# arnauqb/GradABM-JUNE

Hardware: NVIDIA B200
Metric: agent_timesteps_per_sec_fwd_bwd (higher is better)
Workload: dtype f32

## Files before the change

gradabm-june_b200/csrc/gj_kernels.cu:

```cuda
#include <cuda_runtime.h>
#include <math.h>
#include <stdint.h>
#include <stdio.h>
#include <stdlib.h>
#include <string.h>

#include "gj_device.cuh"
#include "gj_tiled.cuh"
#include "gj_lean.cuh"
#include "gj_pipe.cuh"

namespace gj {

static thread_local char g_err[512] = "";

static int fail(const char* what, cudaError_t e) {
  snprintf(g_err, sizeof(g_err), "%s: %s", what, cudaGetErrorString(e));
  return -2;
}
static int bad(const char* what) {
  snprintf(g_err, sizeof(g_err), "invalid argument: %s", what);
  return -1;
}
#define GJ_CHECK_LAUNCH(name)                         \
  do {                                                \
    cudaError_t _e = cudaGetLastError();              \
    if (_e != cudaSuccess) return fail(name, _e);     \
  } while (0)

enum KernelId {
  K_TRANSMISSION = 0, K_GROUP_SMALL_F, K_GROUP_CHUNK_F, K_GROUP_FIX_F, K_AGENT_FWD,
  K_AGENT_BWD, K_GROUP_SMALL_B, K_GROUP_CHUNK_B, K_GROUP_FIX_B, K_DBETA, K_AGENT_BWD_GATHER, K_CELL, K_OTHER, K_SEED,
  K_EXCHANGE, K_SEED_GRAD, K_COUNT
};
static const char* kKernelNames[K_COUNT] = {
  "transmission", "group_small<fwd>", "group_chunk<fwd>", "group_fix<fwd>", "agent_forward",
  "agent_backward", "group_small<bwd>", "group_chunk<bwd>", "group_fix<bwd>", "dbeta",
  "backward_gather", "cell_groups+gather", "other", "seeding", "boundary_exchange", "seed_label_grad"};
constexpr int kMaxProfiled = 16384;
struct Profiler {
  bool on = false;
  int n = 0;
  int64_t launches[K_COUNT] = {0};
  cudaEvent_t ev[kMaxProfiled][2];
  int id[kMaxProfiled];
  bool created = false;
};
static Profiler g_prof;
struct ProfScope {
  int slot = -1;
  cudaStream_t st;
  ProfScope(int kid, cudaStream_t s) : st(s) {
    g_prof.launches[kid]++;
// ... 605 lines not shown
  return (int)(w->n_tiles < g ? w->n_tiles : g);
}

static int g_pipe_on = -1;
static int pipe_flags() {
  if (g_pipe_on < 0) {
    const char* e = getenv("GJ_PIPE");
    g_pipe_on = (e && e[0] >= '0' && e[0] <= '7') ? (e[0] - '0') : 1;
    const char* c = getenv("GJ_K1C");
    if (c && c[0] == '0') g_pipe_on |= 4;
  }
  return g_pipe_on;
}
static bool pipe_enabled() { return (pipe_flags() & 1) != 0; }
static bool lookahead_enabled() { return (pipe_flags() & 3) == 3; }
static bool aligned16(const void* p) { return (((uintptr_t)p) & 15u) == 0; }
static bool pipe_aligned_fwd(const gj_world_desc* w, const LeanPlan& lp, const gj_fwd_io* io) {
  return aligned16(io->s) && aligned16(io->inf) && aligned16(io->tinf) && aligned16(io->cur) && aligned16(io->nxt) &&
         aligned16(io->ttn) && aligned16(io->T) && aligned16(io->Tq) && aligned16(w->ent1) && aligned16(w->cls) &&
         aligned16(w->orig_id) &&
         aligned16(lp.r_slot) && aligned16(lp.r_pc);
}
static bool pipe_aligned_bwd(const gj_world_desc* w, const LeanPlan& lp, const gj_bwd_io* io) {
  const void* ptrs[] = {io->s, io->inf, io->tinf, io->cur, io->nxt, io->ttn, io->tape_y0, io->tape_v, io->g_s_o,
                        io->g_inf_o, io->g_tinf_o, io->g_cur_o, io->g_nxt_o, io->g_ttn_o, io->prof4, io->g_inf,
                        io->g_tinf, io->T_in, io->w, io->wq, w->ent1, w->cls, lp.r_slot, lp.r_pc};
  for (const void* q : ptrs)
    if (!aligned16(q)) return false;
  return true;
}
// ... 35 lines not shown
  if (w->n_chunks > 0) {
    ProfScope ps(kBwd ? K_GROUP_CHUNK_B : K_GROUP_CHUNK_F, st);
    k_group_chunk<kBwd><<<blocks_for(w->n_chunks * 32, kBlock), kBlock, 0, st>>>(*w, *p, ch, beta, lprob, in0, in1,
                                                                              out_a, out_b, sc.part_a, sc.part_b);
    GJ_CHECK_LAUNCH("k_group_chunk");
  }
  if (w->n_big > 0) {
    ProfScope ps(kBwd ? K_GROUP_FIX_B : K_GROUP_FIX_F, st);
    k_group_fix<kBwd><<<blocks_for(w->n_big, kBlock), kBlock, 0, st>>>(*w, *p, ch, beta, sc.part_a, sc.part_b, out_a,
                                                                     out_b);
    GJ_CHECK_LAUNCH("k_group_fix");
  }
  return 0;
}

static int launch_cell_groups(const gj_world_desc* w, const gj_step_params* p, const Plan& pl, const float* beta,
                              float* out_scaled, float* out_plain, const Scratch& sc, cudaStream_t st,
                              const Batch& bt = kNoBatch) {
  if (pl.n_t2 == 0) return 0;
  int64_t maxG = 1;
  for (int j = 0; j < pl.n_t2; ++j) {
    const int t = p->nets[pl.t2_net[j]].type;
    const int64_t G = w->type_group_off[t + 1] - w->type_group_off[t];
    if (G > maxG) maxG = G;
  }
  ProfScope ps(K_CELL, st);
  launch_pdl(k_cell_groups, dim3(blocks_for(maxG, kBlock), pl.n_t2, bt.nb), dim3(kBlock), 0, st, *w, *p, pl, beta,
             (const float*)sc.tile_part, out_scaled, out_plain, bt);
  GJ_CHECK_LAUNCH("k_cell_groups");
  return 0;
}

static int launch_cell_gather(const gj_world_desc* w, const gj_step_params* p, const Plan& pl, const float* in_scaled,
                              const Scratch& sc, cudaStream_t st, const Batch& bt = kNoBatch) {
  if (pl.n_t2 == 0) return 0;
  int64_t maxC = 1;
  for (int j = 0; j < pl.n_t2; ++j) {
    const int t = p->nets[pl.t2_net[j]].type;
    if (w->n_cells[t] > maxC) maxC = w->n_cells[t];
  }
  ProfScope ps(K_CELL, st);
  launch_pdl(k_cell_gather, dim3(blocks_for(maxC, kBlock), pl.n_t2, bt.nb), dim3(kBlock), 0, st, *w, *p, pl, in_scaled,
             sc.cell_buf, bt);
  GJ_CHECK_LAUNCH("k_cell_gather");
  return 0;
}

static bool lean_plan(const gj_world_desc* w, const gj_step_params* p, const Plan& pl, LeanPlan* lp) {
  memset(lp, 0, sizeof(*lp));
  if (p->mode != GJ_MODE_STEP || p->phases != GJ_PHASE_ALL || p->exact_order) return false;
  if (p->n_nets <= 0 || pl.n_t1 > 1) return false;
  if (pl.n_generic > 0 && !w->ent1) return false;
  int64_t total = 0;
  for (int k = 0; k < p->n_nets; ++k) {
    const int kind = p->nets[k].kind, t = p->nets[k].type;
    total += w->type_group_off[t + 1] - w->type_group_off[t];
    if (pl.tier[k] == GJ_TIER_RANGE) {
// ... 20 lines not shown
    } else if (kind == GJ_KIND_HOUSEHOLD) {
      if (p->n_quar > 0) return false;
    } else if (kind != GJ_KIND_PLAIN) {
      return false;
    }
  }
  lp->n_cell = pl.n_t2;
  lp->has_generic = pl.n_generic > 0;
  lp->gen_base = total;
  return true;
}

static int launch_lean_group_pass(const gj_world_desc* w, const gj_step_params* p, const Plan& pl, const float* beta,
                                  const float* in, float* out_scaled, float* out_plain, const Scratch& sc, bool bwd,
                                  cudaStream_t st, const Batch& bt);
static int launch_lean_forward_sums(const gj_world_desc* w, const gj_step_params* p, const Plan& pl, const float* beta,
                                    const float* in, float* out_scaled, float* out_plain, const Scratch& sc,
                                    cudaStream_t st, const Batch& bt) {
  if (w->n_giant_chunks > 0) {
    gj_world_desc wg = *w;
    wg.n_small = 0;
    wg.n_chunks = w->n_giant_chunks;
    wg.n_big = w->n_giant_big;
    if (int e = launch_lean_group_pass(&wg, p, pl, beta, in, out_scaled, out_plain, sc, false, st, bt)) return e;
  }
  {
    ProfScope ps(K_GROUP_SMALL_F, st);
    Scatter sct{sc.sct_acc, sc.sct_dirty};
    GenericRanges gr;
    memset(&gr, 0, sizeof(gr));
    for (int t = 0; t < w->n_types; ++t)
      if (w->type_tier[t] == GJ_TIER_GENERIC && w->type_group_off[t + 1] > w->type_group_off[t]) {
        gr.first[gr.n] = w->type_group_off[t];
        gr.start[gr.n + 1] = gr.start[gr.n] + (w->type_group_off[t + 1] - w->type_group_off[t]);
        ++gr.n;
      }
    if (gr.n == 0) return 0;
    launch_pdl(k_lean_scatter_finalize, dim3(blocks_for(gr.start[gr.n], kBlock) * bt.nb), dim3(kBlock), 0, st, *w, *p, pl,
               gr, beta, in, sct, out_scaled, out_plain, bt);
    GJ_CHECK_LAUNCH("k_lean_scatter_finalize");
  }
  return 0;
}

static int launch_lean_group_pass(const gj_world_desc* w, const gj_step_params* p, const Plan& pl, const float* beta,
                                  const float* in, float* out_scaled, float* out_plain, const Scratch& sc, bool bwd,
                                  cudaStream_t st, const Batch& bt) {
  if (w->n_small > 0 || w->n_chunks > 0) {
    ProfScope ps(bwd ? K_GROUP_CHUNK_B : K_GROUP_CHUNK_F, st);
    const int chunk_blocks = w->n_chunks > 0 ? blocks_for(w->n_chunks * 32, kBlock) : 0;
    const int small_blocks = w->n_small > 0 ? blocks_for(w->n_small, kBlock) : 0;
    launch_pdl(k_lean_group_sums, dim3((chunk_blocks + small_blocks) * bt.nb), dim3(kBlock), 0, st, *w, *p, pl, beta, in,
               out_scaled, out_plain, sc.part_a, chunk_blocks, bt);
    GJ_CHECK_LAUNCH("k_lean_group_sums");
  }
  if (w->n_big > 0) {
    ProfScope ps(bwd ? K_GROUP_FIX_B : K_GROUP_FIX_F, st);
    launch_pdl(k_lean_group_fix, dim3(blocks_for(w->n_big * 32, kBlock) * bt.nb), dim3(kBlock), 0, st, *w, *p, pl, beta,
               (const float*)sc.part_a, out_scaled, out_plain, bt);
    GJ_CHECK_LAUNCH("k_lean_group_fix");
  }
  return 0;
}

static int lean_forward(const gj_world_desc* w, const gj_step_params* p, const Plan& pl, const LeanPlan& lp,
                        const gj_fwd_io* io, const Scratch& sc, cudaStream_t st, const NextStep* next,
                        const Batch& bt = kNoBatch) {
  const bool quar = p->n_quar > 0;
  const bool batch = bt.nb > 1;
  if (p->stage != GJ_STAGE_REST) {
    if (!p->t_ready) {
      ProfScope ps(K_TRANSMISSION, st);
      static OccCache occ[4];
      const Scatter sct{sc.sct_acc, sc.sct_dirty};
#define GJ_K1(Q, B, I)                                                                                               \
  launch_pdl(k_lean_transmission<Q, B>, dim3(lean_grid(w, k_lean_transmission<Q, B>, &occ[I], bt)), dim3(kLeanThreads), \
             0, st, *w, *p, lp, *io, sc.tile_part, sct, bt)
#define GJ_K1C(Q, B, I)                                                                                              \
  launch_pdl(k_lean_transmission_c<Q, B>, dim3(lean_grid(w, k_lean_transmission_c<Q, B>, &occ_c[I], bt)),              \
             dim3(kLeanThreads), 0, st, *w, *p, lp, *io, sc.tile_part, sct, bt)
      static OccCache occ_c[4];
      const bool compact = (pipe_flags() & 4) == 0;
      if (compact) {
        if (batch) {
// ... 2 lines not shown
        } else {
          if (quar) GJ_K1C(true, false, 1);
          else GJ_K1C(false, false, 0);
        }
      } else if (batch) {
        if (quar) GJ_K1(true, true, 3);
        else GJ_K1(false, true, 2);
      } else {
        if (quar) GJ_K1(true, false, 1);
        else GJ_K1(false, false, 0);
      }
#undef GJ_K1
#undef GJ_K1C
      GJ_CHECK_LAUNCH("k_lean_transmission");
    }
    if (lp.has_generic)
      if (int e = launch_lean_forward_sums(w, p, pl, io->beta, quar ? io->Tq : io->T, io->S_scaled + lp.gen_base,
                                           io->S_unscaled + lp.gen_base, sc, st, bt))
        return e;
    if (int e = launch_cell_groups(w, p, pl, io->beta, io->S_scaled, io->S_unscaled, sc, st, bt)) return e;
  }
  if (p->stage == GJ_STAGE_SUMS) return 0;
  if (int e = launch_cell_gather(w, p, pl, io->S_scaled, sc, st, bt)) return e;
  if (batch && bt.noise && pipe_enabled() && pipe_aligned_fwd(w, lp, io)) {
    ProfScope pn(K_OTHER, st);
    launch_pdl(k_batch_noise, dim3(agent_grid(w->n_agents)), dim3(kBlock), 0, st, *w, *p, const_cast<float*>(bt.noise));
    GJ_CHECK_LAUNCH("k_batch_noise");
  }
  if (pipe_enabled() && pipe_aligned_fwd(w, lp, io)) {
    ProfScope ps(K_AGENT_FWD, st);
    static OccCache occ[20];
    const bool diag = io->q || io->n;
    const bool lab = io->label != nullptr;
    const size_t smem = next ? sizeof(PipeFwdSharedT<true, false>)
                             : (batch ? sizeof(PipeFwdSharedT<false, true>) : sizeof(PipeFwdSharedT<false, false>));
    NextStep nx;
    memset(&nx, 0, sizeof(nx));
    if (next) {
// ... 56 lines not shown
    }
#undef GJ_LEAN_FWD
    GJ_CHECK_LAUNCH("k_lean_forward");
  }
  return 0;
}

static int lean_backward(const gj_world_desc* w, const gj_step_params* p, const Plan& pl, LeanPlan lp,
                         const gj_bwd_io* io, const Scratch& sc, cudaStream_t st, const Batch& bt = kNoBatch) {
  const bool quar = p->n_quar > 0;
  const bool batch = bt.nb > 1;
  static OccCache occ_b[4], occ_g[2];
  const bool lab = io->label && io->g_red_label;
  int gather_grid = 1;
  const bool pipe = pipe_enabled() && pipe_aligned_bwd(w, lp, io);
  if (batch && !pipe) return bad("batched step: the pipelined kernels are off or an array is not 16-byte aligned");
  if (p->stage != GJ_STAGE_REST) {
    if (pipe) {
      ProfScope ps(K_AGENT_BWD, st);
      static OccCache occ[8];
      const size_t smem = sizeof(PipeBwdShared);
#define GJ_PIPE_BWD(Q, B, L, I)                                                                                       \
  launch_pdl(k_pipe_backward<Q, B, L>, dim3(pipe_grid(w, k_pipe_backward<Q, B, L>, kBwdThreads, smem, &occ[I], bt)),    \
             dim3(kBwdThreads), smem, st, *w, *p, lp, *io, sc.tile_part, bt)
      if (lab && batch) {
        if (quar) GJ_PIPE_BWD(true, true, true, 7);
        else GJ_PIPE_BWD(false, true, true, 6);
      } else if (lab) {
        if (quar) GJ_PIPE_BWD(true, false, true, 5);
        else GJ_PIPE_BWD(false, false, true, 4);
// ... 8 lines not shown
      GJ_CHECK_LAUNCH("k_pipe_backward");
    } else {
      ProfScope ps(K_AGENT_BWD, st);
#define GJ_LEAN_BWD(Q, L, I) \
  k_lean_backward<Q, L><<<lean_grid(w, k_lean_backward<Q, L>, &occ_b[I]), kLeanThreads, 0, st>>>(*w, *p, lp, *io, sc.tile_part)
      if (lab) {
        if (quar) GJ_LEAN_BWD(true, true, 3);
        else GJ_LEAN_BWD(false, true, 2);
      } else {
        if (quar) GJ_LEAN_BWD(true, false, 1);
        else GJ_LEAN_BWD(false, false, 0);
      }
#undef GJ_LEAN_BWD
      GJ_CHECK_LAUNCH("k_lean_backward");
    }
    if (lp.has_generic)
      if (int e = launch_lean_group_pass(w, p, pl, io->beta, quar ? io->wq : io->w, io->cR + lp.gen_base,
                                         io->R + lp.gen_base, sc, true, st, bt))
        return e;
    if (int e = launch_cell_groups(w, p, pl, io->beta, io->cR, io->R, sc, st, bt)) return e;
  }
  if (p->stage == GJ_STAGE_SUMS) return 0;
  if (int e = launch_cell_gather(w, p, pl, io->cR, sc, st, bt)) return e;
  if (pipe) {
    ProfScope ps(K_AGENT_BWD_GATHER, st);
    static OccCache occ[4];
    const size_t smem = sizeof(PipeGatShared);
#define GJ_PIPE_GAT(Q, B, I)                                                                                          \
  launch_pdl(k_pipe_backward_gather<Q, B>,                                                                            \
             dim3(gather_grid = pipe_grid(w, k_pipe_backward_gather<Q, B>, kPipeThreads, smem, &occ[I], bt)),          \
             dim3(kPipeThreads), smem, st, *w, *p, lp, *io, (const float*)sc.cell_buf, sc.dbeta_tile, bt)
    if (batch) {
      if (quar) GJ_PIPE_GAT(true, true, 3);
      else GJ_PIPE_GAT(false, true, 2);
    } else {
      if (quar) GJ_PIPE_GAT(true, false, 1);
      else GJ_PIPE_GAT(false, false, 0);
    }
// ... 307 lines not shown
  }
  return err ? 1 : 0;
}

int gj_peer_destroy(gj_peer* p) {
  if (!p) return 0;
  for (int r = 0; r < p->world; ++r)
    if (r != p->rank && p->mapped[r]) cudaIpcCloseMemHandle(p->mapped[r]);
  cudaFree(p->own);
  delete p;
  return 0;
}

int gj_pipeline_enable(int on) {
  const int prev = pipe_flags();
  if (on >= 0) g_pipe_on = on & 7;
  return prev;
}

int gj_profile_enable(int on) {
  if (on && !g_prof.created) {
    for (int i = 0; i < kMaxProfiled; ++i) {
      if (cudaEventCreate(&g_prof.ev[i][0]) != cudaSuccess || cudaEventCreate(&g_prof.ev[i][1]) != cudaSuccess)
        return fail("cudaEventCreate", cudaGetLastError());
    }
    g_prof.created = true;
  }
  g_prof.on = on != 0;
  g_prof.n = 0;
  for (int i = 0; i < K_COUNT; ++i) g_prof.launches[i] = 0;
  return 0;
// ... 440 lines not shown
```

gradabm-june_b200/csrc/gj_lean.cuh:

```cuda
#pragma once
#include "gj_tiled.cuh"

namespace gj {

constexpr int kLeanThreads = 256;
#ifndef GJ_LEAN_MINB_FWD
#define GJ_LEAN_MINB_FWD 3
#endif
#ifndef GJ_LEAN_MINB_BWD
#define GJ_LEAN_MINB_BWD 4
#endif
#ifndef GJ_LEAN_MINB_GATHER
#define GJ_LEAN_MINB_GATHER 3
#endif
constexpr uint32_t kEntNone = 0xFFFFFFFFu;
constexpr uint32_t kEntMulti = 0xFFFFFFFEu;
constexpr uint32_t kEntGiant = 0x80000000u;
constexpr uint32_t kEntId = 0x7FFFFFFFu;

struct Scatter {
  unsigned long long* acc;
  uint8_t* dirty;
};
constexpr float kScatterScale = (float)(1ull << GJ_SCATTER_FRAC);
// ... 478 lines not shown
    bx /= (uint32_t)bt.nb;
    beta += (int64_t)s * bt.sBeta;
    in += (int64_t)s * bt.sN;
    out_scaled += (int64_t)s * bt.sG;
    out_plain += (int64_t)s * bt.sG;
    part = scr_shift(part, bt, s);
  }
  lean_beta_sums(gs, w, p, pl, beta);
  if ((int)bx < chunk_blocks)
    lean_group_chunk_body(w, gs, ((int64_t)bx * blockDim.x + threadIdx.x) >> 5, in, out_scaled, out_plain, part);
  else
    lean_group_small_body(w, gs, (int64_t)(bx - chunk_blocks) * blockDim.x + threadIdx.x, in, out_scaled,
                          out_plain);
}

__global__ void __launch_bounds__(kBlock) k_lean_group_fix(gj_world_desc w, gj_step_params p, Plan pl,
                                                           const float* __restrict__ beta,
                                                           const float* __restrict__ part,
                                                           float* __restrict__ out_scaled,
                                                           float* __restrict__ out_plain, Batch bt) {
  __shared__ LeanGroupShared gs;
  pdl_launch();
  pdl_wait();
  uint32_t bx = blockIdx.x;
  if (bt.nb > 1) {
    const int s = (int)(bx % (uint32_t)bt.nb);
    bx /= (uint32_t)bt.nb;
    beta += (int64_t)s * bt.sBeta;
    out_scaled += (int64_t)s * bt.sG;
    out_plain += (int64_t)s * bt.sG;
    part = scr_shift(part, bt, s);
  }
  lean_beta_sums(gs, w, p, pl, beta);
  const int lane = threadIdx.x & 31;
  const int64_t i = ((int64_t)bx * blockDim.x + threadIdx.x) >> 5;
  if (i >= w.n_big) return;
  const uint32_t g = w.big_groups[i];
  const float b = lean_group_beta(gs, g);
  float S = 0.0f;
  for (uint32_t j = w.big_part_ptr[i] + lane; j < w.big_part_ptr[i + 1]; j += 32) S += part[j];
  S = warp_sum(S);
  if (lane != 0) return;
  out_plain[g] = S;
  out_scaled[g] = (b == b) ? (b * w.pc[g]) * S : 0.0f;
}

struct GenericRanges {
  int n;
  int64_t first[GJ_MAX_TYPES];
  int64_t start[GJ_MAX_TYPES + 1];
};
__global__ void __launch_bounds__(kBlock) k_lean_scatter_finalize(gj_world_desc w, gj_step_params p, Plan pl,
                                                                  GenericRanges gr, const float* __restrict__ beta,
                                                                  const float* __restrict__ in, Scatter sct,
                                                                  float* __restrict__ out_scaled,
                                                                  float* __restrict__ out_plain, Batch bt) {
  __shared__ LeanGroupShared gs;
  pdl_launch();
  pdl_wait();
  uint32_t bx = blockIdx.x;
  if (bt.nb > 1) {
    const int s = (int)(bx % (uint32_t)bt.nb);
    bx /= (uint32_t)bt.nb;
    beta += (int64_t)s * bt.sBeta;
    in += (int64_t)s * bt.sN;
    out_scaled += (int64_t)s * bt.sG;
    out_plain += (int64_t)s * bt.sG;
    sct.acc = scr_shift(sct.acc, bt, s);
    sct.dirty = scr_shift(sct.dirty, bt, s);
  }
  lean_beta_sums(gs, w, p, pl, beta);
  const int64_t i = (int64_t)bx * blockDim.x + threadIdx.x;
  if (i >= gr.start[gr.n]) return;
  int r = 0;
#pragma unroll
  for (int k = 1; k < GJ_MAX_TYPES; ++k) r += (k < gr.n && i >= gr.start[k]) ? 1 : 0;
  const int64_t g = gr.first[r] + (i - gr.start[r]);
  const uint32_t j0 = w.gm_ptr[g], j1 = w.gm_ptr[g + 1];
  if (j1 - j0 > (uint32_t)GJ_SCATTER_MAX_GROUP) return;
  const unsigned long long acc = sct.acc[g];
  const bool dirty = sct.dirty[g] != 0;
  if (acc != 0ull) sct.acc[g] = 0ull;
  const float b = lean_group_beta(gs, (uint32_t)g);
  float S = (float)((double)(long long)acc * (1.0 / (double)(1ull << GJ_SCATTER_FRAC)));
  if (dirty) {
    sct.dirty[g] = 0;
    S = 0.0f;
    for (uint32_t j = j0; j < j1; ++j) S += in[w.gm_agent[j]];
  }
  out_plain[g] = S;
  out_scaled[g] = (b == b) ? (b * w.pc[g]) * S : 0.0f;
}

struct FwdOut {
  float inf, tinf, cur;
};
struct FwdRes {
  float tape_v, tape_y0, q, lam, n;
  float s_o, inf_o, tinf_o, cur_o, nxt_o, ttn_o;
};
__device__ __forceinline__ float lean_noise_dE(uint32_t r0, uint32_t r1) {
  return lg2_fast(fmaxf(-lg2_fast(u01_open(r0)), kMinE2)) - lg2_fast(fmaxf(-lg2_fast(u01_open(r1)), kMinE2));
}
template <bool kQuar>
__device__ __forceinline__ FwdRes lean_forward_core(const gj_step_params& p, const LeanPlan& lp,
                                                    const float* __restrict__ stage_prob, uint64_t ga, float dE,
// ... 569 lines not shown
```

gradabm-june_b200/csrc/gj_tiled.cuh:

```cuda
#pragma once
#include "gj_device.cuh"

namespace gj {

constexpr uint32_t kNoSlot = 0xFFFFFFFFu;

struct Plan {
  int n_t2;
  int t2_net[GJ_MAX_CHANNELS];
  int net_t2[GJ_MAX_NETS];
  int n_t1;
  int t1_net[GJ_MAX_RANGE_NETS];
  int net_t1[GJ_MAX_NETS];
  int n_lei;
  int lei_net[GJ_MAX_CHANNELS];
  int net_lei[GJ_MAX_NETS];
  int n_generic;
  int tier[GJ_MAX_NETS];
  const uint32_t* slot[GJ_MAX_NETS];
  const float* rpc[GJ_MAX_NETS];
};

struct Batch {
  int nb;
// ... 141 lines not shown
    float Tq = T;
    if (quar) {
      Tq = quarantine_mask(p, io.cur[a]) * T;
      io.Tq[a] = Tq;
    }
    if (pl.n_t2 > 0 && T != 0.0f) {
      const int cls = w.cls[a];
#pragma unroll
      for (int j = 0; j < GJ_MAX_CHANNELS; ++j)
        if (j < pl.n_t2) acc[j] += member_value(tb, pl, pl.t2_net[j], p.nets[pl.t2_net[j]].kind, T, Tq, cls);
    }
  }
  if (pl.n_t2 > 0) block_sums<float, GJ_MAX_CHANNELS>(acc, pl.n_t2, tile_part + tile * GJ_MAX_CHANNELS);
}

__global__ void __launch_bounds__(kBlock) k_cell_groups(gj_world_desc w, gj_step_params p, Plan pl,
                                                        const float* __restrict__ beta,
                                                        const float* __restrict__ tile_part,
                                                        float* __restrict__ out_scaled, float* __restrict__ out_plain,
                                                        Batch bt) {
  pdl_launch();
  pdl_wait();
  if (bt.nb > 1) {
    const int s = blockIdx.z;
    beta += (int64_t)s * bt.sBeta;
    tile_part = scr_shift(tile_part, bt, s);
    out_scaled += (int64_t)s * bt.sG;
    out_plain += (int64_t)s * bt.sG;
  }
  const int j = blockIdx.y;
  const int k = pl.t2_net[j];
  const gj_net net = p.nets[k];
  const int t = net.type;
  const int64_t G = w.type_group_off[t + 1] - w.type_group_off[t];
  const int64_t g = (int64_t)blockIdx.x * blockDim.x + threadIdx.x;
  if (g >= G) return;
  float sum = 0.0f;
  for (uint32_t ci = w.grp_cell_ptr[t][g]; ci < w.grp_cell_ptr[t][g + 1]; ++ci) {
    const uint32_t c = w.grp_cell[t][ci];
    for (uint32_t tl = w.cell_tile_ptr[t][c]; tl < w.cell_tile_ptr[t][c + 1]; ++tl)
      sum += tile_part[(int64_t)tl * GJ_MAX_CHANNELS + j];
  }
  const float cg = beta[k] * w.pc[w.type_group_off[t] + g];
  out_plain[(int64_t)net.s_off + g] = sum;
  out_scaled[(int64_t)net.s_off + g] = cg * sum;
}

__global__ void __launch_bounds__(kBlock) k_cell_gather(gj_world_desc w, gj_step_params p, Plan pl,
                                                        const float* __restrict__ in_scaled,
                                                        float* __restrict__ cell_buf, Batch bt) {
  pdl_launch();
  pdl_wait();
  if (bt.nb > 1) {
    const int s = blockIdx.z;
    in_scaled += (int64_t)s * bt.sG;
    cell_buf = scr_shift(cell_buf, bt, s);
  }
  const int j = blockIdx.y;
  const gj_net net = p.nets[pl.t2_net[j]];
  const int t = net.type;
  const int64_t c = (int64_t)blockIdx.x * blockDim.x + threadIdx.x;
  if (c >= w.n_cells[t]) return;
  float sum = 0.0f;
  for (uint32_t gi = w.cell_grp_ptr[t][c]; gi < w.cell_grp_ptr[t][c + 1]; ++gi)
    sum += in_scaled[(int64_t)net.s_off + w.cell_grp[t][gi]];
  cell_buf[(w.cell_off[t] + c) * GJ_MAX_CHANNELS + j] = sum;
}

struct AgentState {
  float s, inf, tinf, cur, nxt, ttn;
};

template <bool kLabel = false, bool kSeed = false>
__device__ __forceinline__ void forward_tail(const gj_step_params& p, const gj_fwd_io& io, int64_t N, int64_t a,
                                             int64_t ga, int age, float q, AgentState st, float* red,
                                             uint32_t* lacc = nullptr) {
  const int dead = p.n_stages - 1;
  if (p.mode == GJ_MODE_SEED) q = 1.0f - io.seed_fraction[kSeed ? io.seed_label[a] : 0] * 1.0f;
  float n = 0.0f;
  StepNoise nz;
  nz.E0 = nz.E1 = 1.0f;
// ... 446 lines not shown
```

gradabm-june_b200/grad_june/_lib.py:

```python
import ctypes as C
import os
import subprocess
from pathlib import Path

PKG_DIR = Path(__file__).resolve().parent
CSRC_DIR = PKG_DIR.parent / "csrc"
INCLUDE_DIR = PKG_DIR.parent.parent / "include"
LIB_PATH = Path(os.environ.get("GJ_LIB_PATH") or PKG_DIR / "libgradjune_b200.so")

GJ_MAX_TYPES = 8
GJ_MAX_NETS = 16
GJ_MAX_STAGES = 16
GJ_MAX_QUAR = 4
GJ_MAX_AGE_BINS = 8
GJ_MAX_CHANNELS = 8
GJ_ABI_VERSION = 12

KIND_PLAIN, KIND_HOUSEHOLD, KIND_LEISURE, KIND_CARE_VISIT = 0, 1, 2, 3
PHASE_NETWORKS, PHASE_SAMPLE, PHASE_INFECT, PHASE_SYMPTOMS, PHASE_ALL = 1, 2, 4, 8, 15
MODE_STEP, MODE_SEED = 0, 1
STAGE_ALL, STAGE_SUMS, STAGE_REST = 0, 1, 2

_u32p = C.c_void_p
_f32p = C.c_void_p
# ... 217 lines not shown
        raise GradJuneLibraryError(f"{what} failed ({rc}): {lib().gj_last_error().decode()}")


EXPORTED_SYMBOLS = [
    "gj_abi_version", "gj_last_error", "gj_config", "gj_scratch_bytes", "gj_profile_prepare", "gj_profile_pack",
    "gj_transmission_forward", "gj_transmission_backward", "gj_step_forward", "gj_step_forward_next", "gj_step_backward",
    "gj_step_forward_batch", "gj_step_backward_batch",
    "gj_philox_fill", "gj_philox_fill_at", "gj_step_plan", "gj_philox4x32_10", "gj_philox2x32_10", "gj_profile_enable", "gj_profile_read",
    "gj_profile_kernel_name", "gj_pipeline_enable", "gj_boundary_pack", "gj_boundary_unpack",
    "gj_peer_create", "gj_peer_handle", "gj_peer_connect", "gj_peer_exchange", "gj_peer_status", "gj_peer_destroy",
    "gj_world_build", "gj_world_build_host", "gj_world_descriptor", "gj_world_permutation", "gj_world_last_error",
    "gj_world_destroy", "gj_memcpy",
]


def pipeline_enable(on=True, lookahead=False, uncompacted=False):
    prev = lib().gj_pipeline_enable(-1 if on is None else ((1 if on else 0) | (2 if (on and lookahead) else 0)
                                                           | (4 if uncompacted else 0)))
    return bool(prev & 1), bool(prev & 2), bool(prev & 4)


def profile_enable(on=True):
    check(lib().gj_profile_enable(1 if on else 0), "gj_profile_enable")


def profile_read():
    n = 24
    ms, timed, launches = (C.c_double * n)(), (C.c_int64 * n)(), (C.c_int64 * n)()
    k = lib().gj_profile_read(ms, timed, launches, n)
    if k < 0:
        check(k, "gj_profile_read")
    return {lib().gj_profile_kernel_name(i).decode(): (ms[i], timed[i], launches[i]) for i in range(k)}
```

Before: 21.17 billion.

## Fuse group sums, cell groups and cell gather into one cooperative persistent kernel

Replaces the separate launches for chunked/small group sums, scatter finalize, cell groups, group fix and cell gather with a single cooperative kernel. Work is dispatched over virtual blocks in two phases separated by a grid-wide barrier. Finalize blocks are processed in pairs to overlap their loads. This is meant to cut launch and inter-kernel gaps, at the cost of a software grid barrier and occupancy-limited persistent scheduling. It is enabled by default for non-batched full-stage steps.

```diff
diff --git a/gradabm-june_b200/csrc/gj_kernels.cu b/gradabm-june_b200/csrc/gj_kernels.cu
--- a/gradabm-june_b200/csrc/gj_kernels.cu
+++ b/gradabm-june_b200/csrc/gj_kernels.cu
@@ -31,12 +31,13 @@
 enum KernelId {
   K_TRANSMISSION = 0, K_GROUP_SMALL_F, K_GROUP_CHUNK_F, K_GROUP_FIX_F, K_AGENT_FWD,
   K_AGENT_BWD, K_GROUP_SMALL_B, K_GROUP_CHUNK_B, K_GROUP_FIX_B, K_DBETA, K_AGENT_BWD_GATHER, K_CELL, K_OTHER, K_SEED,
-  K_EXCHANGE, K_SEED_GRAD, K_COUNT
+  K_EXCHANGE, K_SEED_GRAD, K_SUMS_F, K_SUMS_B, K_COUNT
 };
 static const char* kKernelNames[K_COUNT] = {
   "transmission", "group_small<fwd>", "group_chunk<fwd>", "group_fix<fwd>", "agent_forward",
   "agent_backward", "group_small<bwd>", "group_chunk<bwd>", "group_fix<bwd>", "dbeta",
-  "backward_gather", "cell_groups+gather", "other", "seeding", "boundary_exchange", "seed_label_grad"};
+  "backward_gather", "cell_groups+gather", "other", "seeding", "boundary_exchange", "seed_label_grad",
+  "sums<fwd>", "sums<bwd>"};
 constexpr int kMaxProfiled = 16384;
 struct Profiler {
   bool on = false;
@@ -672,6 +673,7 @@
 }
 static bool pipe_enabled() { return (pipe_flags() & 1) != 0; }
 static bool lookahead_enabled() { return (pipe_flags() & 3) == 3; }
+static bool fused_sums_enabled() { return (pipe_flags() & 8) == 0; }
 static bool aligned16(const void* p) { return (((uintptr_t)p) & 15u) == 0; }
 static bool pipe_aligned_fwd(const gj_world_desc* w, const LeanPlan& lp, const gj_fwd_io* io) {
   return aligned16(io->s) && aligned16(io->inf) && aligned16(io->tinf) && aligned16(io->cur) && aligned16(io->nxt) &&
@@ -737,33 +739,40 @@
   return 0;
 }
 
-static int launch_cell_groups(const gj_world_desc* w, const gj_step_params* p, const Plan& pl, const float* beta,
-                              float* out_scaled, float* out_plain, const Scratch& sc, cudaStream_t st,
-                              const Batch& bt = kNoBatch) {
-  if (pl.n_t2 == 0) return 0;
+static int cell_group_blocks(const gj_world_desc* w, const gj_step_params* p, const Plan& pl) {
   int64_t maxG = 1;
   for (int j = 0; j < pl.n_t2; ++j) {
     const int t = p->nets[pl.t2_net[j]].type;
     const int64_t G = w->type_group_off[t + 1] - w->type_group_off[t];
     if (G > maxG) maxG = G;
   }
-  ProfScope ps(K_CELL, st);
-  launch_pdl(k_cell_groups, dim3(blocks_for(maxG, kBlock), pl.n_t2, bt.nb), dim3(kBlock), 0, st, *w, *p, pl, beta,
-             (const float*)sc.tile_part, out_scaled, out_plain, bt);
-  GJ_CHECK_LAUNCH("k_cell_groups");
-  return 0;
-}
-
-static int launch_cell_gather(const gj_world_desc* w, const gj_step_params* p, const Plan& pl, const float* in_scaled,
-                              const Scratch& sc, cudaStream_t st, const Batch& bt = kNoBatch) {
-  if (pl.n_t2 == 0) return 0;
+  return blocks_for(maxG, kBlock);
+}
+static int cell_gather_blocks(const gj_world_desc* w, const gj_step_params* p, const Plan& pl) {
   int64_t maxC = 1;
   for (int j = 0; j < pl.n_t2; ++j) {
     const int t = p->nets[pl.t2_net[j]].type;
     if (w->n_cells[t] > maxC) maxC = w->n_cells[t];
   }
+  return blocks_for(maxC, kBlock);
+}
+
+static int launch_cell_groups(const gj_world_desc* w, const gj_step_params* p, const Plan& pl, const float* beta,
+                              float* out_scaled, float* out_plain, const Scratch& sc, cudaStream_t st,
+                              const Batch& bt = kNoBatch) {
+  if (pl.n_t2 == 0) return 0;
   ProfScope ps(K_CELL, st);
-  launch_pdl(k_cell_gather, dim3(blocks_for(maxC, kBlock), pl.n_t2, bt.nb), dim3(kBlock), 0, st, *w, *p, pl, in_scaled,
+  launch_pdl(k_cell_groups, dim3(cell_group_blocks(w, p, pl), pl.n_t2, bt.nb), dim3(kBlock), 0, st, *w, *p, pl, beta,
+             (const float*)sc.tile_part, out_scaled, out_plain, bt);
+  GJ_CHECK_LAUNCH("k_cell_groups");
+  return 0;
+}
+
+static int launch_cell_gather(const gj_world_desc* w, const gj_step_params* p, const Plan& pl, const float* in_scaled,
+                              const Scratch& sc, cudaStream_t st, const Batch& bt = kNoBatch) {
+  if (pl.n_t2 == 0) return 0;
+  ProfScope ps(K_CELL, st);
+  launch_pdl(k_cell_gather, dim3(cell_gather_blocks(w, p, pl), pl.n_t2, bt.nb), dim3(kBlock), 0, st, *w, *p, pl, in_scaled,
              sc.cell_buf, bt);
   GJ_CHECK_LAUNCH("k_cell_gather");
   return 0;
@@ -814,6 +823,17 @@
 static int launch_lean_group_pass(const gj_world_desc* w, const gj_step_params* p, const Plan& pl, const float* beta,
                                   const float* in, float* out_scaled, float* out_plain, const Scratch& sc, bool bwd,
                                   cudaStream_t st, const Batch& bt);
+static GenericRanges generic_ranges(const gj_world_desc* w) {
+  GenericRanges gr;
+  memset(&gr, 0, sizeof(gr));
+  for (int t = 0; t < w->n_types; ++t)
+    if (w->type_tier[t] == GJ_TIER_GENERIC && w->type_group_off[t + 1] > w->type_group_off[t]) {
+      gr.first[gr.n] = w->type_group_off[t];
+      gr.start[gr.n + 1] = gr.start[gr.n] + (w->type_group_off[t + 1] - w->type_group_off[t]);
+      ++gr.n;
+    }
+  return gr;
+}
 static int launch_lean_forward_sums(const gj_world_desc* w, const gj_step_params* p, const Plan& pl, const float* beta,
                                     const float* in, float* out_scaled, float* out_plain, const Scratch& sc,
                                     cudaStream_t st, const Batch& bt) {
@@ -827,14 +847,7 @@
   {
     ProfScope ps(K_GROUP_SMALL_F, st);
     Scatter sct{sc.sct_acc, sc.sct_dirty};
-    GenericRanges gr;
-    memset(&gr, 0, sizeof(gr));
-    for (int t = 0; t < w->n_types; ++t)
-      if (w->type_tier[t] == GJ_TIER_GENERIC && w->type_group_off[t + 1] > w->type_group_off[t]) {
-        gr.first[gr.n] = w->type_group_off[t];
-        gr.start[gr.n + 1] = gr.start[gr.n] + (w->type_group_off[t + 1] - w->type_group_off[t]);
-        ++gr.n;
-      }
+    const GenericRanges gr = generic_ranges(w);
     if (gr.n == 0) return 0;
     launch_pdl(k_lean_scatter_finalize, dim3(blocks_for(gr.start[gr.n], kBlock) * bt.nb), dim3(kBlock), 0, st, *w, *p, pl,
                gr, beta, in, sct, out_scaled, out_plain, bt);
@@ -863,11 +876,80 @@
   return 0;
 }
 
+constexpr int kSumsBarrier = 62;
+static_assert(1 + GJ_MAX_NETS <= kSumsBarrier && (kSumsBarrier + 2) * sizeof(unsigned int) <= 256,
+              "grid barrier words overlap the reduction tickets");
+static_assert(sizeof(gj_world_desc) + sizeof(gj_step_params) + sizeof(Plan) + sizeof(SumsPlan) <= 32764,
+              "k_lean_sums parameters exceed the 32 KB kernel parameter limit");
+static int launch_lean_sums(const gj_world_desc* w, const gj_step_params* p, const Plan& pl, const LeanPlan& lp,
+                            const float* beta, const float* in, float* scaled, float* plain, const Scratch& sc,
+                            bool bwd, cudaStream_t st) {
+  SumsPlan sp;
+  memset(&sp, 0, sizeof(sp));
+  sp.beta = beta;
+  sp.in = in;
+  sp.gen_scaled = scaled + lp.gen_base;
+  sp.gen_plain = plain + lp.gen_base;
+  sp.part = sc.part_a;
+  if (lp.has_generic) {
+    sp.n_chunks = bwd ? w->n_chunks : w->n_giant_chunks;
+    sp.n_big = bwd ? w->n_big : w->n_giant_big;
+    sp.chunk_blocks = sp.n_chunks > 0 ? blocks_for(sp.n_chunks * 32, kBlock) : 0;
+    sp.small_blocks = (bwd && w->n_small > 0) ? blocks_for(w->n_small, kBlock) : 0;
+    sp.fix_blocks = sp.n_big > 0 ? blocks_for(sp.n_big * 32, kBlock) : 0;
+    if (!bwd) {
+      sp.gr = generic_ranges(w);
+      sp.sct = Scatter{sc.sct_acc, sc.sct_dirty};
+      sp.fin_blocks = sp.gr.n > 0 ? blocks_for(sp.gr.start[sp.gr.n], kBlock) : 0;
+    }
+  }
+  sp.tile_part = sc.tile_part;
+  sp.cell_scaled = scaled;
+  sp.cell_plain = plain;
+  sp.cell_buf = sc.cell_buf;
+  if (pl.n_t2 > 0) {
+    sp.cg_blocks = cell_group_blocks(w, p, pl);
+    sp.cc_blocks = cell_gather_blocks(w, p, pl);
+  }
+  sp.bar = sc.tickets + kSumsBarrier;
+  const int64_t n1 = (int64_t)sp.chunk_blocks + sp.small_blocks + sp.fin_blocks + (int64_t)pl.n_t2 * sp.cg_blocks;
+  const int64_t n2 = (int64_t)sp.fix_blocks + (int64_t)pl.n_t2 * sp.cc_blocks;
+  if (n1 + n2 == 0) return 0;
+  if (n1 >= ((int64_t)1 << 31) || n2 >= ((int64_t)1 << 31)) return bad("too many groups for k_lean_sums");
+  static OccCache occ;
+  int& per_sm = occ.v[current_device()];
+  if (per_sm == 0) {
+    cudaError_t e = cudaOccupancyMaxActiveBlocksPerMultiprocessor(&per_sm, k_lean_sums, kBlock, 0);
+    if (e != cudaSuccess || per_sm < 1) {
+      per_sm = 0;
+      return e != cudaSuccess ? fail("occupancy of k_lean_sums", e) : bad("k_lean_sums does not fit on an SM");
+    }
+  }
+  int64_t grid = (int64_t)sm_count() * per_sm;
+  const int64_t work = n1 > n2 ? n1 : n2;
+  if (grid > work) grid = work;
+  ProfScope ps(bwd ? K_SUMS_B : K_SUMS_F, st);
+  cudaLaunchConfig_t cfg;
+  memset(&cfg, 0, sizeof(cfg));
+  cfg.gridDim = dim3((unsigned)grid);
+  cfg.blockDim = dim3(kBlock);
+  cfg.stream = st;
+  cudaLaunchAttribute attr[1];
+  attr[0].id = cudaLaunchAttributeCooperative;
+  attr[0].val.cooperative = 1;
+  cfg.attrs = attr;
+  cfg.numAttrs = 1;
+  const cudaError_t e = cudaLaunchKernelEx(&cfg, k_lean_sums, *w, *p, pl, sp);
+  if (e != cudaSuccess) return fail("k_lean_sums", e);
+  return 0;
+}
+
 static int lean_forward(const gj_world_desc* w, const gj_step_params* p, const Plan& pl, const LeanPlan& lp,
                         const gj_fwd_io* io, const Scratch& sc, cudaStream_t st, const NextStep* next,
                         const Batch& bt = kNoBatch) {
   const bool quar = p->n_quar > 0;
   const bool batch = bt.nb > 1;
+  const bool fused = fused_sums_enabled() && !batch && p->stage == GJ_STAGE_ALL;
   if (p->stage != GJ_STAGE_REST) {
     if (!p->t_ready) {
       ProfScope ps(K_TRANSMISSION, st);
@@ -900,14 +982,21 @@
 #undef GJ_K1C
       GJ_CHECK_LAUNCH("k_lean_transmission");
     }
-    if (lp.has_generic)
-      if (int e = launch_lean_forward_sums(w, p, pl, io->beta, quar ? io->Tq : io->T, io->S_scaled + lp.gen_base,
-                                           io->S_unscaled + lp.gen_base, sc, st, bt))
+    if (fused) {
+      if (int e = launch_lean_sums(w, p, pl, lp, io->beta, quar ? io->Tq : io->T, io->S_scaled, io->S_unscaled, sc,
+                                   false, st))
         return e;
-    if (int e = launch_cell_groups(w, p, pl, io->beta, io->S_scaled, io->S_unscaled, sc, st, bt)) return e;
+    } else {
+      if (lp.has_generic)
+        if (int e = launch_lean_forward_sums(w, p, pl, io->beta, quar ? io->Tq : io->T, io->S_scaled + lp.gen_base,
+                                             io->S_unscaled + lp.gen_base, sc, st, bt))
+          return e;
+      if (int e = launch_cell_groups(w, p, pl, io->beta, io->S_scaled, io->S_unscaled, sc, st, bt)) return e;
+    }
   }
   if (p->stage == GJ_STAGE_SUMS) return 0;
-  if (int e = launch_cell_gather(w, p, pl, io->S_scaled, sc, st, bt)) return e;
+  if (!fused)
+    if (int e = launch_cell_gather(w, p, pl, io->S_scaled, sc, st, bt)) return e;
   if (batch && bt.noise && pipe_enabled() && pipe_aligned_fwd(w, lp, io)) {
     ProfScope pn(K_OTHER, st);
     launch_pdl(k_batch_noise, dim3(agent_grid(w->n_agents)), dim3(kBlock), 0, st, *w, *p, const_cast<float*>(bt.noise));
@@ -994,6 +1083,7 @@
   const bool lab = io->label && io->g_red_label;
   int gather_grid = 1;
   const bool pipe = pipe_enabled() && pipe_aligned_bwd(w, lp, io);
+  const bool fused = fused_sums_enabled() && !batch && p->stage == GJ_STAGE_ALL;
   if (batch && !pipe) return bad("batched step: the pipelined kernels are off or an array is not 16-byte aligned");
   if (p->stage != GJ_STAGE_REST) {
     if (pipe) {
@@ -1032,14 +1122,20 @@
 #undef GJ_LEAN_BWD
       GJ_CHECK_LAUNCH("k_lean_backward");
     }
-    if (lp.has_generic)
-      if (int e = launch_lean_group_pass(w, p, pl, io->beta, quar ? io->wq : io->w, io->cR + lp.gen_base,
-                                         io->R + lp.gen_base, sc, true, st, bt))
+    if (fused) {
+      if (int e = launch_lean_sums(w, p, pl, lp, io->beta, quar ? io->wq : io->w, io->cR, io->R, sc, true, st))
         return e;
-    if (int e = launch_cell_groups(w, p, pl, io->beta, io->cR, io->R, sc, st, bt)) return e;
+    } else {
+      if (lp.has_generic)
+        if (int e = launch_lean_group_pass(w, p, pl, io->beta, quar ? io->wq : io->w, io->cR + lp.gen_base,
+                                           io->R + lp.gen_base, sc, true, st, bt))
+          return e;
+      if (int e = launch_cell_groups(w, p, pl, io->beta, io->cR, io->R, sc, st, bt)) return e;
+    }
   }
   if (p->stage == GJ_STAGE_SUMS) return 0;
-  if (int e = launch_cell_gather(w, p, pl, io->cR, sc, st, bt)) return e;
+  if (!fused)
+    if (int e = launch_cell_gather(w, p, pl, io->cR, sc, st, bt)) return e;
   if (pipe) {
     ProfScope ps(K_AGENT_BWD_GATHER, st);
     static OccCache occ[4];
@@ -1377,7 +1473,7 @@
 
 int gj_pipeline_enable(int on) {
   const int prev = pipe_flags();
-  if (on >= 0) g_pipe_on = on & 7;
+  if (on >= 0) g_pipe_on = on & 15;
   return prev;
 }
 
diff --git a/gradabm-june_b200/csrc/gj_lean.cuh b/gradabm-june_b200/csrc/gj_lean.cuh
--- a/gradabm-june_b200/csrc/gj_lean.cuh
+++ b/gradabm-june_b200/csrc/gj_lean.cuh
@@ -516,6 +516,20 @@
                           out_plain);
 }
 
+__device__ __forceinline__ void lean_group_fix_body(const gj_world_desc& w, const LeanGroupShared& gs, int64_t i,
+                                                    int64_t n_big, const float* part, float* out_scaled,
+                                                    float* out_plain) {
+  const int lane = threadIdx.x & 31;
+  if (i >= n_big) return;
+  const uint32_t g = w.big_groups[i];
+  const float b = lean_group_beta(gs, g);
+  float S = 0.0f;
+  for (uint32_t j = w.big_part_ptr[i] + lane; j < w.big_part_ptr[i + 1]; j += 32) S += part[j];
+  S = warp_sum(S);
+  if (lane != 0) return;
+  out_plain[g] = S;
+  out_scaled[g] = (b == b) ? (b * w.pc[g]) * S : 0.0f;
+}
 __global__ void __launch_bounds__(kBlock) k_lean_group_fix(gj_world_desc w, gj_step_params p, Plan pl,
                                                            const float* __restrict__ beta,
                                                            const float* __restrict__ part,
@@ -534,17 +548,7 @@
     part = scr_shift(part, bt, s);
   }
   lean_beta_sums(gs, w, p, pl, beta);
-  const int lane = threadIdx.x & 31;
-  const int64_t i = ((int64_t)bx * blockDim.x + threadIdx.x) >> 5;
-  if (i >= w.n_big) return;
-  const uint32_t g = w.big_groups[i];
-  const float b = lean_group_beta(gs, g);
-  float S = 0.0f;
-  for (uint32_t j = w.big_part_ptr[i] + lane; j < w.big_part_ptr[i + 1]; j += 32) S += part[j];
-  S = warp_sum(S);
-  if (lane != 0) return;
-  out_plain[g] = S;
-  out_scaled[g] = (b == b) ? (b * w.pc[g]) * S : 0.0f;
+  lean_group_fix_body(w, gs, ((int64_t)bx * blockDim.x + threadIdx.x) >> 5, w.n_big, part, out_scaled, out_plain);
 }
 
 struct GenericRanges {
@@ -552,6 +556,29 @@
   int64_t first[GJ_MAX_TYPES];
   int64_t start[GJ_MAX_TYPES + 1];
 };
+__device__ __forceinline__ void lean_finalize_body(const gj_world_desc& w, const LeanGroupShared& gs,
+                                                   const GenericRanges& gr, int64_t i, const float* __restrict__ in,
+                                                   const Scatter& sct, float* out_scaled, float* out_plain) {
+  if (i >= gr.start[gr.n]) return;
+  int r = 0;
+#pragma unroll
+  for (int k = 1; k < GJ_MAX_TYPES; ++k) r += (k < gr.n && i >= gr.start[k]) ? 1 : 0;
+  const int64_t g = gr.first[r] + (i - gr.start[r]);
+  const uint32_t j0 = w.gm_ptr[g], j1 = w.gm_ptr[g + 1];
+  if (j1 - j0 > (uint32_t)GJ_SCATTER_MAX_GROUP) return;
+  const unsigned long long acc = sct.acc[g];
+  const bool dirty = sct.dirty[g] != 0;
+  if (acc != 0ull) sct.acc[g] = 0ull;
+  const float b = lean_group_beta(gs, (uint32_t)g);
+  float S = (float)((double)(long long)acc * (1.0 / (double)(1ull << GJ_SCATTER_FRAC)));
+  if (dirty) {
+    sct.dirty[g] = 0;
+    S = 0.0f;
+    for (uint32_t j = j0; j < j1; ++j) S += in[w.gm_agent[j]];
+  }
+  out_plain[g] = S;
+  out_scaled[g] = (b == b) ? (b * w.pc[g]) * S : 0.0f;
+}
 __global__ void __launch_bounds__(kBlock) k_lean_scatter_finalize(gj_world_desc w, gj_step_params p, Plan pl,
                                                                   GenericRanges gr, const float* __restrict__ beta,
                                                                   const float* __restrict__ in, Scatter sct,
@@ -572,26 +599,150 @@
     sct.dirty = scr_shift(sct.dirty, bt, s);
   }
   lean_beta_sums(gs, w, p, pl, beta);
-  const int64_t i = (int64_t)bx * blockDim.x + threadIdx.x;
-  if (i >= gr.start[gr.n]) return;
-  int r = 0;
-#pragma unroll
-  for (int k = 1; k < GJ_MAX_TYPES; ++k) r += (k < gr.n && i >= gr.start[k]) ? 1 : 0;
-  const int64_t g = gr.first[r] + (i - gr.start[r]);
-  const uint32_t j0 = w.gm_ptr[g], j1 = w.gm_ptr[g + 1];
-  if (j1 - j0 > (uint32_t)GJ_SCATTER_MAX_GROUP) return;
-  const unsigned long long acc = sct.acc[g];
-  const bool dirty = sct.dirty[g] != 0;
-  if (acc != 0ull) sct.acc[g] = 0ull;
-  const float b = lean_group_beta(gs, (uint32_t)g);
-  float S = (float)((double)(long long)acc * (1.0 / (double)(1ull << GJ_SCATTER_FRAC)));
-  if (dirty) {
-    sct.dirty[g] = 0;
-    S = 0.0f;
-    for (uint32_t j = j0; j < j1; ++j) S += in[w.gm_agent[j]];
-  }
-  out_plain[g] = S;
-  out_scaled[g] = (b == b) ? (b * w.pc[g]) * S : 0.0f;
+  lean_finalize_body(w, gs, gr, (int64_t)bx * blockDim.x + threadIdx.x, in, sct, out_scaled, out_plain);
+}
+
+#ifndef GJ_SUMS_MINB
+#define GJ_SUMS_MINB 8
+#endif
+struct SumsPlan {
+  const float* beta;
+  const float* in;
+  float* gen_scaled;
+  float* gen_plain;
+  float* part;
+  int64_t n_chunks, n_big;
+  int chunk_blocks, small_blocks, fin_blocks, fix_blocks;
+  GenericRanges gr;
+  Scatter sct;
+  const float* tile_part;
+  float* cell_scaled;
+  float* cell_plain;
+  float* cell_buf;
+  int cg_blocks, cc_blocks;
+  unsigned int* bar;
+};
+
+__device__ __forceinline__ void grid_barrier(unsigned int* bar) {
+  __syncthreads();
+  if (threadIdx.x == 0) {
+    volatile unsigned int* gen = bar + 1;
+    const unsigned int g = *gen;
+    __threadfence();
+    if (atomicAdd(bar, 1u) == gridDim.x - 1u) {
+      atomicExch(bar, 0u);
+      __threadfence();
+      atomicAdd(bar + 1, 1u);
+    } else {
+      unsigned long long t0, t1;
+      asm volatile("mov.u64 %0, %%globaltimer;" : "=l"(t0));
+      while (*gen == g) {
+        __nanosleep(64);
+        asm volatile("mov.u64 %0, %%globaltimer;" : "=l"(t1));
+        if (t1 - t0 > 10000000000ull) __trap();
+      }
+    }
+    __threadfence();
+  }
+  __syncthreads();
+}
+
+__device__ __forceinline__ void sums_phase1_block(const gj_world_desc& w, const gj_step_params& p, const Plan& pl,
+                                                  const SumsPlan& sp, const LeanGroupShared& gs, int b) {
+  if (b < sp.chunk_blocks) {
+    const int64_t ci = ((int64_t)b * kBlock + threadIdx.x) >> 5;
+    if (ci < sp.n_chunks) lean_group_chunk_body(w, gs, ci, sp.in, sp.gen_scaled, sp.gen_plain, sp.part);
+    return;
+  }
+  b -= sp.chunk_blocks;
+  if (b < sp.small_blocks) {
+    lean_group_small_body(w, gs, (int64_t)b * kBlock + threadIdx.x, sp.in, sp.gen_scaled, sp.gen_plain);
+    return;
+  }
+  b -= sp.small_blocks;
+  if (b < sp.fin_blocks) {
+    lean_finalize_body(w, gs, sp.gr, (int64_t)b * kBlock + threadIdx.x, sp.in, sp.sct, sp.gen_scaled, sp.gen_plain);
+    return;
+  }
+  b -= sp.fin_blocks;
+  const int j = b / sp.cg_blocks;
+  cell_group_body(w, p, pl, j, (int64_t)(b - j * sp.cg_blocks) * kBlock + threadIdx.x, sp.beta, sp.tile_part,
+                  sp.cell_scaled, sp.cell_plain);
+}
+
+__device__ __forceinline__ void lean_finalize_pair(const gj_world_desc& w, const LeanGroupShared& gs,
+                                                   const GenericRanges& gr, int64_t i0, int64_t i1,
+                                                   const float* __restrict__ in, const Scatter& sct, float* out_scaled,
+                                                   float* out_plain) {
+  const int64_t i[2] = {i0, i1};
+  int64_t g[2];
+  bool on[2];
+  uint32_t n[2];
+  unsigned long long acc[2];
+  bool dirty[2];
+  float pc[2];
+#pragma unroll
+  for (int h = 0; h < 2; ++h) {
+    on[h] = i[h] < gr.start[gr.n];
+    int r = 0;
+#pragma unroll
+    for (int k = 1; k < GJ_MAX_TYPES; ++k) r += (k < gr.n && i[h] >= gr.start[k]) ? 1 : 0;
+    g[h] = on[h] ? gr.first[r] + (i[h] - gr.start[r]) : 0;
+  }
+#pragma unroll
+  for (int h = 0; h < 2; ++h) {
+    n[h] = on[h] ? w.gm_ptr[g[h] + 1] - w.gm_ptr[g[h]] : 0u;
+    acc[h] = on[h] ? sct.acc[g[h]] : 0ull;
+    dirty[h] = on[h] && sct.dirty[g[h]] != 0;
+    pc[h] = on[h] ? w.pc[g[h]] : 0.0f;
+  }
+#pragma unroll
+  for (int h = 0; h < 2; ++h) {
+    if (!on[h] || n[h] > (uint32_t)GJ_SCATTER_MAX_GROUP) continue;
+    if (acc[h] != 0ull) sct.acc[g[h]] = 0ull;
+    const float b = lean_group_beta(gs, (uint32_t)g[h]);
+    float S = (float)((double)(long long)acc[h] * (1.0 / (double)(1ull << GJ_SCATTER_FRAC)));
+    if (dirty[h]) {
+      sct.dirty[g[h]] = 0;
+      S = 0.0f;
+      for (uint32_t j = w.gm_ptr[g[h]]; j < w.gm_ptr[g[h] + 1]; ++j) S += in[w.gm_agent[j]];
+    }
+    out_plain[g[h]] = S;
+    out_scaled[g[h]] = (b == b) ? (b * pc[h]) * S : 0.0f;
+  }
+}
+
+__global__ void __launch_bounds__(kBlock, GJ_SUMS_MINB) k_lean_sums(gj_world_desc w, gj_step_params p, Plan pl,
+                                                                    SumsPlan sp) {
+  __shared__ LeanGroupShared gs;
+  lean_beta_sums(gs, w, p, pl, sp.beta);
+  const int n1 = sp.chunk_blocks + sp.small_blocks + sp.fin_blocks + pl.n_t2 * sp.cg_blocks;
+  const int s_fin = sp.chunk_blocks + sp.small_blocks, s_cell = s_fin + sp.fin_blocks;
+  for (int vb = blockIdx.x; vb < n1; vb += 2 * gridDim.x) {
+    const int vb2 = vb + gridDim.x;
+    if (vb >= s_fin && vb2 < s_cell) {
+      lean_finalize_pair(w, gs, sp.gr, (int64_t)(vb - s_fin) * kBlock + threadIdx.x,
+                         (int64_t)(vb2 - s_fin) * kBlock + threadIdx.x, sp.in, sp.sct, sp.gen_scaled,
+                         sp.gen_plain);
+    } else {
+      sums_phase1_block(w, p, pl, sp, gs, vb);
+      if (vb2 < n1) sums_phase1_block(w, p, pl, sp, gs, vb2);
+    }
+  }
+  const int n2 = sp.fix_blocks + pl.n_t2 * sp.cc_blocks;
+  if (n2 == 0) return;
+  if (n1 > 0) grid_barrier(sp.bar);
+  for (int vb = blockIdx.x; vb < n2; vb += gridDim.x) {
+    int b = vb;
+    if (b < sp.fix_blocks) {
+      lean_group_fix_body(w, gs, ((int64_t)b * kBlock + threadIdx.x) >> 5, sp.n_big, sp.part, sp.gen_scaled,
+                          sp.gen_plain);
+      continue;
+    }
+    b -= sp.fix_blocks;
+    const int j = b / sp.cc_blocks;
+    cell_gather_body(w, p, pl, j, (int64_t)(b - j * sp.cc_blocks) * kBlock + threadIdx.x, sp.cell_scaled, sp.cell_buf);
+  }
 }
 
 struct FwdOut {
diff --git a/gradabm-june_b200/csrc/gj_tiled.cuh b/gradabm-june_b200/csrc/gj_tiled.cuh
--- a/gradabm-june_b200/csrc/gj_tiled.cuh
+++ b/gradabm-june_b200/csrc/gj_tiled.cuh
@@ -179,6 +179,24 @@
   if (pl.n_t2 > 0) block_sums<float, GJ_MAX_CHANNELS>(acc, pl.n_t2, tile_part + tile * GJ_MAX_CHANNELS);
 }
 
+__device__ __forceinline__ void cell_group_body(const gj_world_desc& w, const gj_step_params& p, const Plan& pl, int j,
+                                                int64_t g, const float* beta, const float* tile_part,
+                                                float* out_scaled, float* out_plain) {
+  const int k = pl.t2_net[j];
+  const gj_net net = p.nets[k];
+  const int t = net.type;
+  const int64_t G = w.type_group_off[t + 1] - w.type_group_off[t];
+  if (g >= G) return;
+  float sum = 0.0f;
+  for (uint32_t ci = w.grp_cell_ptr[t][g]; ci < w.grp_cell_ptr[t][g + 1]; ++ci) {
+    const uint32_t c = w.grp_cell[t][ci];
+    for (uint32_t tl = w.cell_tile_ptr[t][c]; tl < w.cell_tile_ptr[t][c + 1]; ++tl)
+      sum += tile_part[(int64_t)tl * GJ_MAX_CHANNELS + j];
+  }
+  const float cg = beta[k] * w.pc[w.type_group_off[t] + g];
+  out_plain[(int64_t)net.s_off + g] = sum;
+  out_scaled[(int64_t)net.s_off + g] = cg * sum;
+}
 __global__ void __launch_bounds__(kBlock) k_cell_groups(gj_world_desc w, gj_step_params p, Plan pl,
                                                         const float* __restrict__ beta,
                                                         const float* __restrict__ tile_part,
@@ -193,24 +211,20 @@
     out_scaled += (int64_t)s * bt.sG;
     out_plain += (int64_t)s * bt.sG;
   }
-  const int j = blockIdx.y;
-  const int k = pl.t2_net[j];
-  const gj_net net = p.nets[k];
+  cell_group_body(w, p, pl, blockIdx.y, (int64_t)blockIdx.x * blockDim.x + threadIdx.x, beta, tile_part, out_scaled,
+                  out_plain);
+}
+
+__device__ __forceinline__ void cell_gather_body(const gj_world_desc& w, const gj_step_params& p, const Plan& pl, int j,
+                                                 int64_t c, const float* in_scaled, float* cell_buf) {
+  const gj_net net = p.nets[pl.t2_net[j]];
   const int t = net.type;
-  const int64_t G = w.type_group_off[t + 1] - w.type_group_off[t];
-  const int64_t g = (int64_t)blockIdx.x * blockDim.x + threadIdx.x;
-  if (g >= G) return;
+  if (c >= w.n_cells[t]) return;
   float sum = 0.0f;
-  for (uint32_t ci = w.grp_cell_ptr[t][g]; ci < w.grp_cell_ptr[t][g + 1]; ++ci) {
-    const uint32_t c = w.grp_cell[t][ci];
-    for (uint32_t tl = w.cell_tile_ptr[t][c]; tl < w.cell_tile_ptr[t][c + 1]; ++tl)
-      sum += tile_part[(int64_t)tl * GJ_MAX_CHANNELS + j];
-  }
-  const float cg = beta[k] * w.pc[w.type_group_off[t] + g];
-  out_plain[(int64_t)net.s_off + g] = sum;
-  out_scaled[(int64_t)net.s_off + g] = cg * sum;
-}
-
+  for (uint32_t gi = w.cell_grp_ptr[t][c]; gi < w.cell_grp_ptr[t][c + 1]; ++gi)
+    sum += in_scaled[(int64_t)net.s_off + w.cell_grp[t][gi]];
+  cell_buf[(w.cell_off[t] + c) * GJ_MAX_CHANNELS + j] = sum;
+}
 __global__ void __launch_bounds__(kBlock) k_cell_gather(gj_world_desc w, gj_step_params p, Plan pl,
                                                         const float* __restrict__ in_scaled,
                                                         float* __restrict__ cell_buf, Batch bt) {
@@ -221,15 +235,7 @@
     in_scaled += (int64_t)s * bt.sG;
     cell_buf = scr_shift(cell_buf, bt, s);
   }
-  const int j = blockIdx.y;
-  const gj_net net = p.nets[pl.t2_net[j]];
-  const int t = net.type;
-  const int64_t c = (int64_t)blockIdx.x * blockDim.x + threadIdx.x;
-  if (c >= w.n_cells[t]) return;
-  float sum = 0.0f;
-  for (uint32_t gi = w.cell_grp_ptr[t][c]; gi < w.cell_grp_ptr[t][c + 1]; ++gi)
-    sum += in_scaled[(int64_t)net.s_off + w.cell_grp[t][gi]];
-  cell_buf[(w.cell_off[t] + c) * GJ_MAX_CHANNELS + j] = sum;
+  cell_gather_body(w, p, pl, blockIdx.y, (int64_t)blockIdx.x * blockDim.x + threadIdx.x, in_scaled, cell_buf);
 }
 
 struct AgentState {
diff --git a/gradabm-june_b200/grad_june/_lib.py b/gradabm-june_b200/grad_june/_lib.py
--- a/gradabm-june_b200/grad_june/_lib.py
+++ b/gradabm-june_b200/grad_june/_lib.py
@@ -255,10 +255,10 @@
 ]
 
 
-def pipeline_enable(on=True, lookahead=False, uncompacted=False):
+def pipeline_enable(on=True, lookahead=False, uncompacted=False, unfused=False):
     prev = lib().gj_pipeline_enable(-1 if on is None else ((1 if on else 0) | (2 if (on and lookahead) else 0)
-                                                           | (4 if uncompacted else 0)))
-    return bool(prev & 1), bool(prev & 2), bool(prev & 4)
+                                                           | (4 if uncompacted else 0) | (8 if unfused else 0)))
+    return bool(prev & 1), bool(prev & 2), bool(prev & 4), bool(prev & 8)
 
 
 def profile_enable(on=True):
```

New measurement: 21.52 billion, median of 6. +1.7%, better.
